# XUANTIE-RV/csi-nn2

Measured on AMD Instinct MI355X. Metric: mobilenetv1_int8_images_per_sec, higher is better.
Workload: dtype i8; 1 GPU; mobilenetv1 int8 NHWC batch 1/GPU, 28 conv layers in 15 launches, hipGraph replay via csinn_*; ops_per_image=1137480704, algorithmic_bytes_per_image=8323144, algorithmic_bytes_per_image_survey=14444616, parallelism=replicas x1

## Files before the change

csi-nn2_amd/__init__.py:

```python
import ctypes as C
import os

import numpy as np

HERE = os.path.dirname(os.path.abspath(__file__))
ROOT = os.path.dirname(HERE)
LIB_DIR = os.path.join(HERE, "lib")

DTYPE_INT8, DTYPE_INT32, DTYPE_FLOAT16, DTYPE_FLOAT32 = 3, 7, 8, 10
MEM_CPU, MEM_DMABUF, MEM_CPU_ACC = 0, 2, 5
QUANT_INT8_ASYM_W_SYM, QUANT_FLOAT16 = 11, 7
API_REF, API_GREF, API_MI355X = 0, 1, 14
RM_LAYER, RM_CPU_GRAPH = 0, 1
LAYOUT_N, LAYOUT_NC, LAYOUT_NCHW, LAYOUT_O, LAYOUT_OI, LAYOUT_OIHW, LAYOUT_O1HW = 1, 2, 4, 6, 7, 11, 13
LAYOUT_NHWC, LAYOUT_OHWI, LAYOUT_1HWO = 15, 18, 22
CSINN_TRUE = 1
OP_CONV2D, OP_CONV2D_RELU, OP_CONV2D_RELU6 = 28, 29, 30
OP_DEPTHWISE_CONV2D, OP_FULLYCONNECTED = 35, 71
OP_AVGPOOL2D, OP_MAXPOOL2D = 14, 98
OP_CONCAT = 26
OP_SPLIT, OP_SHUFFLE_CHANNEL = 166, 153
OP_SIGMOID, OP_HARD_SIGMOID, OP_SILU, OP_LEAKY_RELU, OP_MUL = 154, 78, 190, 84, 107
OP_RESIZE = 133
OP_DECONV2D, OP_DEPTHWISE_DECONV2D, OP_GROUP_DECONV2D = 54, 55, 56
# ... 158 lines not shown
                ("a_zp", C.c_int32), ("b_zp", C.c_int32), ("out_zp", C.c_int32), ("a_is_second", C.c_int32),
                ("reserved", C.c_int32 * 4)]


ABI_STRUCTS = {"csinn_quant_info": QuantInfo, "csinn_tensor": Tensor, "csinn_session": Session,
               "csinn_callback": Callback, "csinn_params_base": ParamsBase,
               "csinn_conv2d_params": Conv2dParams, "csinn_fc_params": FcParams,
               "csinn_relu_params": ReluParams, "csinn_model": Model,
               "csinn_softmax_params": SoftmaxParams, "csinn_pool_params": PoolParams,
               "csinn_diso_params": DisoParams}


def lib_path(name):
    return os.path.join(LIB_DIR, name)


_loaded = {}


def _cdll(path, mode=C.RTLD_GLOBAL):
    if path not in _loaded:
        if not os.path.exists(path):
            raise MI355XError("native library missing: %s (run python csi-nn2_amd/build.py)" % path)
        _loaded[path] = C.CDLL(path, mode=mode)
    return _loaded[path]


def load_hip():
    lib = _cdll(lib_path("libshl_mi355x.so"))
    if getattr(lib, "_typed", False):
        return lib
    vp, sz, i32, f32 = C.c_void_p, C.c_size_t, C.c_int32, C.c_float
    sigs = {
        "shl_mi355x_abi_version": (C.c_int, []),
        "shl_mi355x_last_error": (C.c_char_p, []),
        "shl_mi355x_device_count": (C.c_int, []),
        "shl_mi355x_set_device": (C.c_int, [C.c_int]),
        "shl_mi355x_device_info": (C.c_int, [C.c_char_p, sz, C.POINTER(i32), C.POINTER(C.c_int64)]),
        "shl_mi355x_malloc": (vp, [sz]),
        "shl_mi355x_free": (C.c_int, [vp]),
        "shl_mi355x_is_device_ptr": (C.c_int, [vp]),
        "shl_mi355x_upload": (C.c_int, [vp, vp, sz, vp]),
        "shl_mi355x_download": (C.c_int, [vp, vp, sz, vp]),
        "shl_mi355x_copy": (C.c_int, [vp, vp, sz, vp]),
        "shl_mi355x_memset": (C.c_int, [vp, C.c_int, sz, vp]),
        "shl_mi355x_stream_create": (vp, []),
        "shl_mi355x_stream_destroy": (C.c_int, [vp]),
        "shl_mi355x_stream_sync": (C.c_int, [vp]),
        "shl_mi355x_event_create": (vp, []),
        "shl_mi355x_event_destroy": (C.c_int, [vp]),
        "shl_mi355x_event_record": (C.c_int, [vp, vp]),
        "shl_mi355x_event_elapsed_ms": (C.c_int, [vp, vp, C.POINTER(f32)]),
        "shl_mi355x_graph_begin": (C.c_int, [vp]),
        "shl_mi355x_graph_end": (vp, [vp]),
        "shl_mi355x_graph_launch": (C.c_int, [vp, vp]),
        "shl_mi355x_graph_destroy": (C.c_int, [vp]),
        "shl_mi355x_conv_plan_create": (C.c_int, [C.POINTER(ConvDesc), vp, vp, vp, vp, C.POINTER(vp)]),
        "shl_mi355x_conv_plan_create_wzp": (C.c_int, [C.POINTER(ConvDesc), vp, vp, vp, vp, vp, C.POINTER(vp)]),
        "shl_mi355x_conv_plan_create_dw_channel": (C.c_int, [C.POINTER(ConvDesc), vp, vp, vp, vp, f32, f32, vp, C.POINTER(vp)]),
        "shl_mi355x_deconv_plan_create": (C.c_int, [C.POINTER(ConvDesc), vp, vp, vp, vp, C.POINTER(vp)]),
        "shl_mi355x_deconv_kernel_name": (C.c_char_p, [C.POINTER(ConvDesc)]),
        "shl_mi355x_deconv_geometry": (C.c_int, [C.POINTER(ConvDesc), C.POINTER(i32), i32]),
        "shl_mi355x_debug_trace": (C.c_int, [vp, i32]),
        "shl_mi355x_debug_div_check": (C.c_int, [vp, i32, vp, vp]),
        "shl_mi355x_debug_f16_round_check": (C.c_int, [vp]),
        "shl_mi355x_debug_mfma_rate": (C.c_int, [i32, i32, C.POINTER(C.c_double), C.POINTER(C.c_double)]),
        "shl_mi355x_comm_available": (C.c_int, []),
        "shl_mi355x_comm_unique_id": (C.c_int, [vp]),
        "shl_mi355x_comm_create": (C.c_int, [vp, i32, i32, C.POINTER(vp)]),
        "shl_mi355x_comm_destroy": (C.c_int, [vp]),
        "shl_mi355x_comm_info": (C.c_int, [vp, C.POINTER(i32), C.POINTER(i32), C.POINTER(i32)]),
        "shl_mi355x_device_bus_id": (C.c_int, [C.c_char_p, sz]),
        "shl_mi355x_comm_bcast": (C.c_int, [vp, C.POINTER(vp), C.POINTER(sz), i32, i32, vp]),
        "shl_mi355x_conv_plan_destroy": (C.c_int, [vp]),
        "shl_mi355x_conv_plan_algo": (C.c_int, [vp]),
        "shl_mi355x_conv_plan_kernel_name": (C.c_char_p, [vp]),
        "shl_mi355x_conv_plan_bytes": (sz, [vp]),
        "shl_mi355x_conv_plan_const_block": (vp, [vp, C.POINTER(sz)]),
        "shl_mi355x_conv_plan_adopt_block": (C.c_int, [vp, vp]),
        "shl_mi355x_conv_forward": (C.c_int, [vp, vp, vp, i32, vp]),
        "shl_mi355x_pwdw_fusable": (C.c_int, [vp, vp, i32]),
        "shl_mi355x_pwdw_form": (C.c_int, [vp, vp, i32]),
        "shl_mi355x_pwdw_geometry": (C.c_int, [vp, vp, i32, C.POINTER(i32), i32]),
        "shl_mi355x_pool_conv_fusable": (C.c_int, [vp, i32, i32]),
        "shl_mi355x_pool_conv_forward": (C.c_int, [vp, vp, vp, i32, i32, f32, i32, f32, i32, vp]),
        "shl_mi355x_conv_pool_fusable": (C.c_int, [vp, i32]),
        "shl_mi355x_conv_pool_forward": (C.c_int, [vp, vp, vp, vp, i32, f32, i32, f32, i32, vp]),
        "shl_mi355x_conv_plan_set_no_stream_consumer": (C.c_int, [vp, i32]),
        "shl_mi355x_pwdw_forward": (C.c_int, [vp, vp, vp, vp, i32, vp]),
        "shl_mi355x_relu_i8": (C.c_int, [vp, vp, sz, f32, i32, f32, i32, i32, vp]),
        "shl_mi355x_relu_f16": (C.c_int, [vp, vp, sz, i32, vp]),
        "shl_mi355x_add": (C.c_int, [vp, vp, vp, sz, i32, f32, i32, f32, i32, f32, i32, vp]),
        "shl_mi355x_layout_convert": (C.c_int, [vp, vp, C.c_int64, i32, i32, i32, i32, vp]),
        "shl_mi355x_global_avgpool2d": (C.c_int, [vp, vp, i32, i32, i32, i32, i32, f32, i32, f32, i32, vp]),
        "shl_mi355x_softmax": (C.c_int, [vp, vp, i32, C.c_int64, i32, C.c_int64, f32, i32, f32, i32, vp]),
        "shl_mi355x_pool2d": (C.c_int, [vp, vp, C.POINTER(PoolDesc), vp]),
        "shl_mi355x_pool2d_kernel_name": (C.c_char_p, [C.POINTER(PoolDesc)]),
        "shl_mi355x_concat": (C.c_int, [C.POINTER(vp), C.POINTER(C.c_int64), C.POINTER(f32), C.POINTER(i32), vp,
                                        C.POINTER(ConcatDesc), vp]),
        "shl_mi355x_concat_kernel_name": (C.c_char_p, [C.POINTER(vp), C.POINTER(C.c_int64), C.POINTER(f32), C.POINTER(i32),
                                                       vp, C.POINTER(ConcatDesc)]),
        "shl_mi355x_split": (C.c_int, [vp, C.POINTER(vp), C.POINTER(C.c_int64), C.POINTER(f32), C.POINTER(i32),
                                       C.POINTER(SplitDesc), vp]),
        "shl_mi355x_split_kernel_name": (C.c_char_p, [vp, C.POINTER(vp), C.POINTER(C.c_int64), C.POINTER(f32), C.POINTER(i32),
                                                      C.POINTER(SplitDesc)]),
        "shl_mi355x_shuffle_channel": (C.c_int, [vp, vp, C.POINTER(ShuffleDesc), vp]),
        "shl_mi355x_shuffle_channel_kernel_name": (C.c_char_p, [vp, vp, C.POINTER(ShuffleDesc)]),
        "shl_mi355x_unary_lut_i8": (C.c_int, [vp, vp, sz, vp, vp]),
        "shl_mi355x_unary_lut_i8_kernel_name": (C.c_char_p, [vp, vp]),
        "shl_mi355x_unary_f16": (C.c_int, [vp, vp, sz, i32, f32, vp]),
        "shl_mi355x_mul": (C.c_int, [vp, vp, vp, C.POINTER(MulDesc), vp]),
        "shl_mi355x_mul_kernel_name": (C.c_char_p, [C.POINTER(MulDesc), vp, vp, vp]),
        "shl_mi355x_resize": (C.c_int, [vp, vp, C.POINTER(ResizeDesc), vp]),
        "shl_mi355x_resize_kernel_name": (C.c_char_p, [C.POINTER(ResizeDesc), vp, vp]),
    }
    for name, (res, args) in sigs.items():
        fn = getattr(lib, name)
        fn.restype, fn.argtypes = res, args
    lib._typed = True
    lib.EXPORTS = sorted(sigs)
    return lib


_FRONTEND_SIGS = {
    "csinn_alloc_session": (C.POINTER(Session), []),
    "csinn_free_session": (None, [C.POINTER(Session)]),
    "csinn_session_init": (None, [C.POINTER(Session)]),
    "csinn_session_deinit": (None, [C.POINTER(Session)]),
    "csinn_session_setup": (C.c_int, [C.POINTER(Session)]),
    "csinn_session_run": (C.c_int, [C.POINTER(Session)]),
    "csinn_set_input_number": (None, [C.c_int, C.POINTER(Session)]),
    "csinn_set_output_number": (None, [C.c_int, C.POINTER(Session)]),
    "csinn_set_input": (C.c_int, [C.c_int, C.POINTER(Tensor), C.POINTER(Session)]),
    "csinn_set_output": (C.c_int, [C.c_int, C.POINTER(Tensor), C.POINTER(Session)]),
    "csinn_get_output": (C.c_int, [C.c_int, C.POINTER(Tensor), C.POINTER(Session)]),
    "csinn_update_input": (C.c_int, [C.c_int, C.POINTER(Tensor), C.POINTER(Session)]),
    "csinn_update_output": (C.c_int, [C.c_int, C.POINTER(Tensor), C.POINTER(Session)]),
    "csinn_set_tensor_entry": (C.c_int, [C.POINTER(Tensor), C.POINTER(Session)]),
    "csinn_alloc_tensor": (C.POINTER(Tensor), [C.POINTER(Session)]),
    "csinn_free_tensor": (None, [C.POINTER(Tensor)]),
    "csinn_alloc_params": (C.c_void_p, [C.c_int, C.POINTER(Session)]),
    "csinn_free_params": (None, [C.c_void_p]),
    "csinn_tensor_size": (C.c_int, [C.POINTER(Tensor)]),
    "csinn_tensor_byte_size": (C.c_int, [C.POINTER(Tensor)]),
    "shl_register_op_callback": (None, [C.c_int, C.c_void_p]),
    "shl_register_runtime_callback": (None, [C.c_int, C.c_void_p]),
    "shl_mem_alloc": (C.c_void_p, [C.c_int64]),
    "shl_mem_free": (None, [C.c_void_p]),
    "shl_debug_set_level": (None, [C.c_int]),
}
_SISO_OPS = ("csinn_relu", "csinn_relu6", "csinn_global_avgpool2d", "csinn_softmax", "csinn_maxpool2d", "csinn_avgpool2d",
             "csinn_sigmoid", "csinn_hard_sigmoid", "csinn_silu", "csinn_leaky_relu", "csinn_resize", "csinn_shuffle_channel")
_CONV_OPS = ["csinn_conv2d", "csinn_conv2d_relu", "csinn_conv2d_relu6", "csinn_depthwise_conv2d",
             "csinn_depthwise_conv2d_relu", "csinn_fullyconnected", "csinn_deconv2d"] + list(_SISO_OPS)


def load_frontend(kind="standalone", local=False, path=None):
    mode = C.RTLD_LOCAL if local else C.RTLD_GLOBAL
    if path is not None:
        lib = _cdll(path, mode)
        kind = "external"
    elif kind == "standalone":
        lib = _cdll(lib_path("libcsinn_nn2.so"), mode)
    else:
        raise ValueError(kind)
    if getattr(lib, "_typed", False):
# ... 266 lines not shown
```

csi-nn2_amd/csrc/common.h:

```cpp
#pragma once

#include <hip/hip_runtime.h>
#include <stdint.h>

#include "shl_mi355x.h"

namespace shl {

typedef int v4i __attribute__((ext_vector_type(4)));
typedef int v16i __attribute__((ext_vector_type(16)));
typedef float v16f __attribute__((ext_vector_type(16)));
typedef _Float16 v8h __attribute__((ext_vector_type(8)));

struct ConvArgs {
    const void *in;
    const void *w;
    void *out;
    const int32_t *acc_init;
    const float *mult;
    const float *bias;
    int32_t N, H, W, C;
    int32_t Ho, Wo, Co;
    int32_t Kh, Kw;
    int32_t sh, sw, pt, pl, dh, dw;
// ... 370 lines not shown
    const float c[4] = {v0, v1, v2, v3};
    uint32_t pk[8];
    finish16_f16_unit_scale<4, 0>(c, [&](int) { return bias_f; }, act, pk);
    return make_uint2(pk[0], pk[1]);
}

void set_error(const char *fmt, ...);
int hip_fail(hipError_t e, const char *what);
#define SHL_HIP(expr)                                          \
    do {                                                       \
        hipError_t e_ = (expr);                                \
        if (e_ != hipSuccess) return shl::hip_fail(e_, #expr); \
    } while (0)

struct LdsOptIn {
    unsigned long long done = 0;
};
inline void lds_opt_in(LdsOptIn &st, const void *kernel, int bytes = 160 * 1024)
{
    int dev = 0;
    if (hipGetDevice(&dev) != hipSuccess) return;
    const unsigned long long bit = 1ull << (dev & 63);
    if (__atomic_load_n(&st.done, __ATOMIC_ACQUIRE) & bit) return;
    const hipError_t e = hipFuncSetAttribute(kernel, hipFuncAttributeMaxDynamicSharedMemorySize, bytes);
    if (e != hipSuccess) {
        hip_fail(e, "hipFuncSetAttribute(MaxDynamicSharedMemorySize)");
        return;
    }
    __atomic_fetch_or(&st.done, bit, __ATOMIC_RELEASE);
}

int launch_conv_direct(const ConvArgs &a, int dtype, int layout, int dw_nhwc_weights,
                       hipStream_t s);
int launch_conv_group_direct(const ConvArgs &a, int dtype, int layout, hipStream_t s);
int launch_conv_igemm(const ConvArgs &a, int dtype, int layout, hipStream_t s);
int launch_dwconv(const ConvArgs &a, int dtype, int layout, hipStream_t s);
bool igemm_supports(const shl_mi355x_conv_desc &d);
const char *igemm_variant(int64_t M, int64_t Co, int64_t kbytes = 0);
const char *igemm_pick_name(const ConvArgs &a, int esize);
bool igemm_fuses_nchw_out(const ConvArgs &a, int esize);
bool dwconv_supports(const shl_mi355x_conv_desc &d);
bool dwconv_dot4_supports(const shl_mi355x_conv_desc &d);
void dwconv_dot4_pack(const shl_mi355x_conv_desc &d, const int8_t *hwo, uint32_t *dst);
bool dwconv_mfma_pick(int64_t M, int C, int H, int W, int Ho, int Wo, int sh, int sw);
int launch_dwconv_mfma(const ConvArgs &a, hipStream_t s);
bool conv1x1_resident_pick(const ConvArgs &a);
int launch_conv1x1_resident(const ConvArgs &a, hipStream_t s);
bool conv1x1_latency_pick(const ConvArgs &a);
int launch_conv1x1_latency(const ConvArgs &a, hipStream_t s);
bool conv1x1_pool_fusable(const ConvArgs &a);
int launch_conv1x1_pool(const ConvArgs &a, void *pool_out, float si, float zi, float so, float zo, int store_map, hipStream_t s);
bool conv1x1_stream_pick(const ConvArgs &a);
int launch_conv1x1_stream(const ConvArgs &a, hipStream_t s);
int launch_dwconv_channel(const ConvArgs &a, hipStream_t s);
bool conv_gemv_pick(const ConvArgs &a, int esize);
int launch_conv_gemv(const ConvArgs &a, int dtype, hipStream_t s);
bool pool_gemv_pick(const ConvArgs &a, int hw);
int launch_pool_gemv(const ConvArgs &a, int hw, float in_scale, int in_zp, float mid_scale, int mid_zp, hipStream_t s);
bool stem_supports(const shl_mi355x_conv_desc &d);
void stem_pack_weights(const shl_mi355x_conv_desc &d, const int8_t *ohwi, int32_t *dst);
size_t stem_weight_bytes(const shl_mi355x_conv_desc &d);
int launch_conv_stem(const ConvArgs &a, hipStream_t s);
bool conv1x1_nchw_eligible(const ConvArgs &a);
int launch_conv1x1_nchw(const ConvArgs &a, int dtype, hipStream_t s);
bool dwconv_nchw_supports(const shl_mi355x_conv_desc &d);
int launch_dwconv_nchw(const ConvArgs &a, int dtype, hipStream_t s);
bool pwdw_fusable(const ConvArgs &pw, const ConvArgs &dw, int pw_is_igemm, int dw_dot4_packed);
int launch_pwdw_fused(const ConvArgs &pw, const ConvArgs &dw, hipStream_t s);
constexpr int SHL_PWDW_GEOMETRY_FIELDS = 12;
bool pwdw_fused_geometry(const ConvArgs &pw, const ConvArgs &dw, int32_t out[SHL_PWDW_GEOMETRY_FIELDS]);
bool stemdw_f16_nchw_fusable(const ConvArgs &stem, const ConvArgs &dw);
int launch_stemdw_f16_nchw(const ConvArgs &stem, const ConvArgs &dw, hipStream_t s);
bool stem_mfma_pick(const ConvArgs &a);
bool dwpw_stream_fusable(const ConvArgs &dw, const ConvArgs &pw, int dw_dot4_packed, int pw_is_igemm);
bool dwpw_stream_takes(const ConvArgs &dw);
int launch_dwpw_stream(const ConvArgs &dw, const ConvArgs &pw, hipStream_t s);
bool dwpw_resident_fusable(const ConvArgs &dw, const ConvArgs &pw, int dw_dot4_packed, int pw_is_igemm);
bool dwpw_resident_takes(const ConvArgs &dw);
int launch_dwpw_resident(const ConvArgs &dw, const ConvArgs &pw, hipStream_t s);
bool pwdw_f16_nchw_fusable(const ConvArgs &pw, const ConvArgs &dw);
int launch_pwdw_f16_nchw(const ConvArgs &pw, const ConvArgs &dw, hipStream_t s);
bool stemdw_fusable(const ConvArgs &stem, const ConvArgs &dw);
int launch_stemdw_fused(const ConvArgs &stem, const ConvArgs &dw, hipStream_t s);
bool patch_supports(const shl_mi355x_conv_desc &d);
int patch_choose_geom(const shl_mi355x_conv_desc &d, int32_t batch);
size_t patch_weight_bytes(const shl_mi355x_conv_desc &d, int geom);
void patch_pack_weights(const shl_mi355x_conv_desc &d, int geom, const int8_t *src, int8_t *dst);
bool patch_setup(ConvArgs &a);
bool patch_auto(const ConvArgs &a, bool vs_wave = false);
int launch_conv_igemm_patch(const ConvArgs &a, hipStream_t s);
enum { DECONV_GATHER = 0, DECONV_PHASE = 1 };
const char *deconv_invalid(const shl_mi355x_conv_desc *d, int *status);
int deconv_form(const shl_mi355x_conv_desc &d, bool epilogue_ok, const char **why);
const char *deconv_form_name(int form, int dtype);
int deconv_phases(const shl_mi355x_conv_desc &d);
size_t deconv_phase_weight_bytes(const shl_mi355x_conv_desc &d);
size_t deconv_phase_acc_bytes(const shl_mi355x_conv_desc &d);
void deconv_pack_phase(const shl_mi355x_conv_desc &d, const char *ohwi, char *dst, int32_t *acc);
int launch_deconv_gather(const ConvArgs &a, int dtype, int layout, hipStream_t s);
int launch_deconv_phase(const ConvArgs &a, const shl_mi355x_conv_desc &d, hipStream_t s);
int launch_transpose(const void *src, void *dst, int64_t n, int R, int S, int esize, hipStream_t s, int to_nhwc);

}
```

csi-nn2_amd/csrc/conv_plan.hip:

```cpp
#include <stdlib.h>
#include <string.h>

#include <map>
#include <mutex>
#include <vector>

#include "igemm_common.h"

struct shl_mi355x_conv_plan {
    shl_mi355x_conv_desc desc;
    int algo;
    char *block;
    size_t block_bytes;
    size_t off_w, off_acc, off_mult, off_bias, off_pad;
    size_t off_wfrag;
    size_t off_wpatch;
    size_t off_flags;
    int32_t pt_geom;
    int32_t div_exact, div_fma, act_clamp;
    float clamp_lo, clamp_hi, inv_out_scale;
    char *scratch_in, *scratch_out;
    int2 *pix_tab;
    float ch_in_scale, ch_out_scale;
    int32_t ch_has_bias;
// ... 1044 lines not shown
    if (a.M == 0) return SHL_MI355X_OK;
    return launch_pool_gemv(a, pixels, in_scale, in_zp, mid_scale, mid_zp, (hipStream_t)stream);
}

int shl_mi355x_conv_pool_fusable(const shl_mi355x_conv_plan *plan, int32_t batch)
{
    using namespace shl;
    if (!plan || batch <= 0) return 0;
    const char *sel = getenv("SHL_MI355X_CONVPOOL");
    if (sel && sel[0] == '0') return 0;
    if (plan->desc.dtype != SHL_MI355X_I8 || plan->desc.layout != SHL_MI355X_NHWC || plan->algo != SHL_MI355X_ALGO_IGEMM) return 0;
    if (igemm_env_override()) return 0;
    ConvArgs a;
    static char dummy[16];
    if (fill_args(plan, dummy, dummy, batch, a) != SHL_MI355X_OK) return 0;
    return conv1x1_pool_fusable(a) ? 1 : 0;
}

int shl_mi355x_conv_pool_forward(const shl_mi355x_conv_plan *plan, const void *input_dev, void *map_dev, void *pool_dev, int32_t batch,
                                 float mid_scale, int32_t mid_zp, float out_scale, int32_t out_zp, void *stream)
{
    using namespace shl;
    if (!plan || !input_dev || !pool_dev) {
        set_error("conv_pool_forward: NULL argument");
        return SHL_MI355X_EINVAL;
    }
    if (!shl_mi355x_conv_pool_fusable(plan, batch)) {
        set_error("conv_pool_forward: the pair does not qualify for the fused kernel");
        return SHL_MI355X_ENOTSUP;
    }
    ConvArgs a;
    static char dummy[16];
    int rc = fill_args(plan, input_dev, map_dev ? map_dev : dummy, batch, a);
    if (rc != SHL_MI355X_OK) return rc;
    if (a.M == 0) return SHL_MI355X_OK;
    return launch_conv1x1_pool(a, pool_dev, mid_scale, (float)mid_zp, out_scale, (float)out_zp, map_dev ? 1 : 0, (hipStream_t)stream);
}

int shl_mi355x_pwdw_form(const shl_mi355x_conv_plan *pw, const shl_mi355x_conv_plan *dw, int32_t batch)
{
    if (!dw || !pw || is_deconv(pw) || is_deconv(dw)) return 0;
    static const char *off = getenv("SHL_MI355X_NO_FUSION");
    static const char *sel = getenv("SHL_MI355X_PWDW");
    if ((off && off[0] == '1') || (sel && sel[0] == '0')) return 0;
    if (dw->desc.dtype != pw->desc.dtype || dw->desc.layout != pw->desc.layout) return 0;
    const bool i8_nhwc = pw->desc.dtype == SHL_MI355X_I8 && pw->desc.layout == SHL_MI355X_NHWC;
    const bool f16_nchw = pw->desc.dtype == SHL_MI355X_F16 && pw->desc.layout == SHL_MI355X_NCHW;
    if (!i8_nhwc && !f16_nchw) return 0;
    ConvArgs a, b;
    static char dummy[16];
    if (fill_args(pw, dummy, dummy, batch, a) != SHL_MI355X_OK || fill_args(dw, dummy, dummy, batch, b) != SHL_MI355X_OK)
        return 0;
    return pwdw_kernel_for(pw, dw, a, b);
}

int shl_mi355x_pwdw_fusable(const shl_mi355x_conv_plan *pw, const shl_mi355x_conv_plan *dw, int32_t batch)
{
    return shl_mi355x_pwdw_form(pw, dw, batch) ? 1 : 0;
}

int shl_mi355x_pwdw_geometry(const shl_mi355x_conv_plan *pw, const shl_mi355x_conv_plan *dw, int32_t batch, int32_t *out, int32_t count)
{
    using namespace shl;
    if (!out || count < SHL_PWDW_GEOMETRY_FIELDS) {
        set_error("pwdw_geometry: room for 12 values is needed");
        return SHL_MI355X_EINVAL;
    }
    if (shl_mi355x_pwdw_form(pw, dw, batch) != 1) {
        set_error("pwdw_geometry: the pair does not run the latency form");
        return SHL_MI355X_ENOTSUP;
    }
    ConvArgs a, b;
    static char dummy[16];
    int rc = fill_args(pw, dummy, dummy, batch, a);
    if (rc == SHL_MI355X_OK) rc = fill_args(dw, dummy, dummy, batch, b);
    if (rc != SHL_MI355X_OK) return rc;
    if (!pwdw_fused_geometry(a, b, out)) {
        set_error("pwdw_geometry: the pair does not qualify");
        return SHL_MI355X_ENOTSUP;
    }
    return SHL_MI355X_OK;
}

int shl_mi355x_pwdw_forward(const shl_mi355x_conv_plan *pw, const shl_mi355x_conv_plan *dw, const void *input_dev,
                            void *output_dev, int32_t batch, void *stream)
{
    if (!dw || !pw || !input_dev || !output_dev) {
        set_error("pwdw_forward: NULL argument");
        return SHL_MI355X_EINVAL;
    }
    if (!shl_mi355x_pwdw_fusable(pw, dw, batch)) {
        set_error("pwdw_forward: the pair does not qualify for the fused kernel");
        return SHL_MI355X_ENOTSUP;
    }
    ConvArgs a, b;
    int rc = fill_args(pw, input_dev, output_dev, batch, a);
    if (rc == SHL_MI355X_OK) rc = fill_args(dw, input_dev, output_dev, batch, b);
    if (rc != SHL_MI355X_OK) return rc;
    if (b.M == 0) return SHL_MI355X_OK;
    switch (pwdw_kernel_for(pw, dw, a, b)) {
        case 7: return launch_dwpw_resident(a, b, (hipStream_t)stream);
        case 6: return launch_dwpw_stream(a, b, (hipStream_t)stream);
        case 5: return launch_stemdw_f16_nchw(a, b, (hipStream_t)stream);
        case 4: return launch_pwdw_f16_nchw(a, b, (hipStream_t)stream);
        case 3: return launch_stemdw_fused(a, b, (hipStream_t)stream);
        default: return launch_pwdw_fused(a, b, (hipStream_t)stream);
    }
}

}
```

csi-nn2_amd/csrc/stemdw_fused.hip:

```cpp
#include <stdio.h>
#include <stdlib.h>

#include "dw_patch.h"

namespace shl {

struct StemDwArgs {
    ConvArgs st;
    ConvArgs dw;
    int32_t bh, bw;
    int32_t tiles_x, tiles_y;
    int32_t rw, npx;
    uint32_t rw_magic, bw_magic;
};

template <int EPQ, int EPD>
__global__ __launch_bounds__(256) void stemdw_fused_kernel(StemDwArgs f)
{
    extern __shared__ __attribute__((aligned(16))) char smem[];
    const ConvArgs &q = f.st;
    const ConvArgs &d = f.dw;
    asm volatile("" ::"s"(q.in), "s"(q.w), "s"(q.acc_init), "s"(q.mult), "s"(q.bias), "s"(q.H), "s"(q.W), "s"(q.Ho), "s"(q.Wo), "s"(q.sh),
                 "s"(q.sw), "s"(q.pt), "s"(q.pl), "s"(q.dh), "s"(q.dw), "s"(q.in_zp));
    asm volatile("" ::"s"(f.bh), "s"(f.bw), "s"(f.tiles_y), "s"(f.rw), "s"(f.npx), "s"(f.rw_magic), "s"(f.bw_magic), "s"(d.N), "s"(d.sh),
                 "s"(d.sw), "s"(d.pt), "s"(d.pl), "s"(d.w), "s"(d.acc_init), "s"(d.mult), "s"(d.bias), "s"(d.out));
    asm volatile("" ::"s"(q.out_zp), "s"(q.out_zp_f), "s"(q.clamp_lo), "s"(q.clamp_hi), "s"(d.out_zp), "s"(d.out_zp_f), "s"(d.clamp_lo),
                 "s"(d.clamp_hi), "s"(d.in_zp), "s"(d.Ho), "s"(d.Wo), "s"(d.H), "s"(d.W), "s"(d.C));
    const int tid = threadIdx.x;
    int32_t *w_lds = reinterpret_cast<int32_t *>(smem);
    int32_t *t_tab = w_lds + 7 * 32;
    uint32_t *patch = reinterpret_cast<uint32_t *>(t_tab + 96);
    if (tid < 224) w_lds[tid] = static_cast<const int32_t *>(q.w)[tid];
    if (tid < 96) {
        const int which = tid >> 5, i = tid & 31;
        t_tab[tid] = which == 0 ? q.acc_init[i] : which == 1 ? __float_as_int(q.mult[i]) : __float_as_int(q.bias[i]);
    }
    const int tx = blockIdx.x;
    int ty = blockIdx.y, n = 0;
    if (d.N > 1) {
        n = ty / f.tiles_y;
        ty -= n * f.tiles_y;
    }
    const int oy0 = ty * f.bh, ox0 = tx * f.bw;
    const int ry0 = oy0 * d.sh - d.pt, rx0 = ox0 * d.sw - d.pl;
    const DwThreadConsts dwk = dw_load_consts(d, 0, tid);

    const int8_t *img = static_cast<const int8_t *>(q.in) + (int64_t)n * q.H * q.W * 3;
    const int ntasks = 2 * f.npx;
    const int ppitch = dw_patch_pitch(f.npx);
    const uint32_t zpad = dw_patch_pad(d);
    DwPatchGeom g;
    g.bh = f.bh, g.bw = f.bw, g.rw = f.rw, g.bw_magic = f.bw_magic, g.pitch = ppitch;
    g.lbh = min(f.bh, d.Ho - oy0), g.lbw = min(f.bw, d.Wo - ox0);
    g.oy0 = oy0, g.ox0 = ox0, g.ry0 = ry0, g.rx0 = rx0, g.n = n, g.ch0 = 0;
    const DwPrep dwp = dw_patch_prepare(d, g, tid);
    for (int base = 0; base < ntasks; base += 256) {
        const bool valid = base + tid < ntasks;
        const int task = valid ? base + tid : ntasks - 1;
        const int j = task >> 1, cb = (task & 1) * 16;
        const int pr = (int)(((uint32_t)j * f.rw_magic) >> 20);
        const int pc = j - pr * f.rw;
        const int sy = ry0 + pr, sx = rx0 + pc;
        const bool inside = (unsigned)sy < (unsigned)q.Ho && (unsigned)sx < (unsigned)q.Wo;
        const int y0 = sy * q.sh - q.pt, x0 = sx * q.sw - q.pl;
        int qv[28];
#pragma unroll
        for (int ky = 0; ky < 3; ++ky)
#pragma unroll
            for (int kx = 0; kx < 3; ++kx) {
                const int y = y0 + ky * q.dh, x = x0 + kx * q.dw;
                const bool ok = inside && (unsigned)y < (unsigned)q.H && (unsigned)x < (unsigned)q.W;
                const int8_t *px = img + ((int64_t)y * q.W + x) * 3;
#pragma unroll
                for (int c = 0; c < 3; ++c) qv[(ky * 3 + kx) * 3 + c] = ok ? (int)px[c] : q.in_zp;
            }
        qv[27] = 0;
        uint32_t q4[7];
#pragma unroll
        for (int g = 0; g < 7; ++g)
            q4[g] = (uint32_t)(qv[4 * g] & 0xFF) | ((uint32_t)(qv[4 * g + 1] & 0xFF) << 8) |
                    ((uint32_t)(qv[4 * g + 2] & 0xFF) << 16) | ((uint32_t)(qv[4 * g + 3] & 0xFF) << 24);
        if (base == 0) __syncthreads();
        int acc[16];
#pragma unroll
        for (int e = 0; e < 16; ++e) acc[e] = 0;
#pragma unroll
        for (int g = 0; g < 7; ++g)
#pragma unroll
            for (int v = 0; v < 4; ++v) {
                const int4 w = *reinterpret_cast<const int4 *>(&w_lds[g * 32 + cb + 4 * v]);
                acc[4 * v + 0] = __builtin_amdgcn_sdot4((int)q4[g], w.x, acc[4 * v + 0], false);
                acc[4 * v + 1] = __builtin_amdgcn_sdot4((int)q4[g], w.y, acc[4 * v + 1], false);
                acc[4 * v + 2] = __builtin_amdgcn_sdot4((int)q4[g], w.z, acc[4 * v + 2], false);
                acc[4 * v + 3] = __builtin_amdgcn_sdot4((int)q4[g], w.w, acc[4 * v + 3], false);
            }
#pragma unroll
        for (int v = 0; v < 4; ++v) {
            const int c = cb + 4 * v;
            const int4 ai = *reinterpret_cast<const int4 *>(t_tab + c);
            const float4 mu = *reinterpret_cast<const float4 *>(t_tab + 32 + c);
            const float4 bi = *reinterpret_cast<const float4 *>(t_tab + 64 + c);
            const uint32_t pk = requant4_i8_sel<EPQ>(acc[4 * v] + ai.x, acc[4 * v + 1] + ai.y, acc[4 * v + 2] + ai.z,
                                               acc[4 * v + 3] + ai.w, mu, bi, q);
            if (valid) patch[dw_patch_slot(j, c >> 2, ppitch)] = inside ? pk : zpad;
        }
    }
    __syncthreads();

    depthwise_from_patch<EPD>(d, patch, g, dwk, dwp, tid, 256);
}

static bool stemdw_geometry(const ConvArgs &q, const ConvArgs &d, StemDwArgs &f)
{
    if (q.Kh != 3 || q.Kw != 3 || q.C != 3 || q.Co != 32) return false;
    if (d.Kh != 3 || d.Kw != 3 || d.dh != 1 || d.dw != 1 || d.C != 32 || d.Co != 32) return false;
    if (d.H != q.Ho || d.W != q.Wo || d.N != q.N || d.sh < 1 || d.sh > 2 || d.sw < 1 || d.sw > 2) return false;
    if (d.pt < 0 || d.pl < 0 || d.pt > 2 || d.pl > 2) return false;
    if ((int64_t)d.Ho * d.Wo * d.C >= ((int64_t)1 << 31)) return false;
    f.bh = d.Ho < 2 ? d.Ho : 2;
    f.bw = d.Wo < 28 ? d.Wo : 28;
    if (const char *e = getenv("SHL_MI355X_STEMDW_TILE")) {
        int h = 0, w = 0;
        if (sscanf(e, "%dx%d", &h, &w) == 2 && h > 0 && w > 0) f.bh = h < d.Ho ? h : d.Ho, f.bw = w < d.Wo ? w : d.Wo;
    }
    f.tiles_y = (d.Ho + f.bh - 1) / f.bh;
    f.tiles_x = (d.Wo + f.bw - 1) / f.bw;
    f.rw = (f.bw - 1) * d.sw + 3;
    f.npx = ((f.bh - 1) * d.sh + 3) * f.rw;
    f.rw_magic = ((1u << 20) + f.rw - 1) / f.rw;
    f.bw_magic = ((1u << 20) + f.bw - 1) / f.bw;
    if (f.npx >= 2048 || f.tiles_x > 65535 || (int64_t)f.tiles_y * d.N > 65535) return false;
    return (int64_t)f.tiles_x * f.tiles_y * d.N <= 2048;
}

bool stemdw_fusable(const ConvArgs &q, const ConvArgs &d)
{
    StemDwArgs f;
    return stemdw_geometry(q, d, f);
}

int launch_stemdw_fused(const ConvArgs &q, const ConvArgs &d, hipStream_t s)
{
    StemDwArgs f;
    f.st = q;
    f.dw = d;
    if (!stemdw_geometry(q, d, f)) {
        set_error("stemdw_fused: the pair does not qualify");
        return SHL_MI355X_ENOTSUP;
    }
    const dim3 grid((unsigned)f.tiles_x, (unsigned)(f.tiles_y * d.N));
    const size_t lds = (size_t)(7 * 32 + 96) * 4 + dw_patch_bytes(f.npx);
    const int epq = (q.act != SHL_MI355X_ACT_NONE && !q.act_clamp) ? -1 : (q.div_exact ? 3 : 0);
    const int epd = (d.act != SHL_MI355X_ACT_NONE && !d.act_clamp) ? -1 : (d.div_exact ? 3 : 0);
    if (epq == 3 && epd == 3) hipLaunchKernelGGL((stemdw_fused_kernel<3, 3>), grid, dim3(256), lds, s, f);
    else if (epq == 0 && epd == 0) hipLaunchKernelGGL((stemdw_fused_kernel<0, 0>), grid, dim3(256), lds, s, f);
    else hipLaunchKernelGGL((stemdw_fused_kernel<-1, -1>), grid, dim3(256), lds, s, f);
    SHL_HIP(hipGetLastError());
    return SHL_MI355X_OK;
}

}
```

include/shl_mi355x.h:

```cpp
#ifndef SHL_MI355X_H_
#define SHL_MI355X_H_

#include <stddef.h>
#include <stdint.h>

#ifdef __cplusplus
extern "C" {
#endif

#define SHL_MI355X_ABI_VERSION 1

enum shl_mi355x_status {
    SHL_MI355X_OK = 0,
    SHL_MI355X_ENODEV = -1,
    SHL_MI355X_EINVAL = -2,
    SHL_MI355X_ENOTSUP = -3,
    SHL_MI355X_EHIP = -4,
    SHL_MI355X_ENOMEM = -5
};

enum shl_mi355x_layout {
    SHL_MI355X_NHWC = 0,
    SHL_MI355X_NCHW = 1
};
// ... 42 lines not shown

typedef struct shl_mi355x_conv_plan shl_mi355x_conv_plan;

int shl_mi355x_abi_version(void);
const char *shl_mi355x_last_error(void);
int shl_mi355x_device_count(void);
int shl_mi355x_set_device(int ordinal);
int shl_mi355x_device_info(char *arch, size_t arch_len, int32_t *cu_count, int64_t *hbm_bytes);
int shl_mi355x_device_bus_id(char *buf, size_t len);

void *shl_mi355x_malloc(size_t bytes);
int shl_mi355x_free(void *ptr_dev);
int shl_mi355x_is_device_ptr(const void *ptr);
int shl_mi355x_upload(void *dst_dev, const void *src_host, size_t bytes, void *stream);
int shl_mi355x_download(void *dst_host, const void *src_dev, size_t bytes, void *stream);
int shl_mi355x_copy(void *dst_dev, const void *src_dev, size_t bytes, void *stream);
int shl_mi355x_memset(void *dst_dev, int byte_value, size_t bytes, void *stream);
void *shl_mi355x_stream_create(void);
int shl_mi355x_stream_destroy(void *stream);
int shl_mi355x_stream_sync(void *stream);

void *shl_mi355x_event_create(void);
int shl_mi355x_event_destroy(void *event);
int shl_mi355x_event_record(void *event, void *stream);
int shl_mi355x_event_elapsed_ms(void *start, void *stop, float *ms);

int shl_mi355x_graph_begin(void *stream);
void *shl_mi355x_graph_end(void *stream);
int shl_mi355x_graph_launch(void *graph_exec, void *stream);
int shl_mi355x_graph_destroy(void *graph_exec);


int shl_mi355x_conv_plan_create(const struct shl_mi355x_conv_desc *desc,
                                const void *kernel_host, const float *mult_host,
                                const float *bias_host, void *stream,
                                shl_mi355x_conv_plan **plan_out);
int shl_mi355x_conv_plan_create_wzp(const struct shl_mi355x_conv_desc *desc, const void *kernel_host,
                                    const float *mult_host, const float *bias_host, const int32_t *kernel_zp,
                                    void *stream, shl_mi355x_conv_plan **plan_out);
int shl_mi355x_comm_available(void);
int shl_mi355x_comm_unique_id(void *id128);
int shl_mi355x_comm_create(const void *id128, int32_t rank, int32_t world, void **comm_out);
int shl_mi355x_comm_destroy(void *comm);
int shl_mi355x_comm_info(void *comm, int32_t *nranks, int32_t *rank, int32_t *device);
int shl_mi355x_comm_bcast(void *comm, void *const *blocks_dev, const size_t *bytes, int32_t count, int32_t root,
                          void *stream);

int shl_mi355x_debug_trace(uint64_t *host, int32_t count);

int shl_mi355x_debug_div_check(const float *divisors_host, int32_t n, uint64_t *mismatches, float *first_pair);
int shl_mi355x_debug_f16_round_check(uint64_t *out3);
int shl_mi355x_debug_mfma_rate(int32_t form, int32_t waves_per_simd, double *tops, double *ns_per_mfma);

int shl_mi355x_conv_plan_create_dw_channel(const struct shl_mi355x_conv_desc *desc, const void *kernel_host,
                                           const float *kernel_scale, const int32_t *kernel_zp,
                                           const int32_t *bias_i32, float in_scale, float out_scale_ms,
                                           void *stream, shl_mi355x_conv_plan **plan_out);

int shl_mi355x_deconv_plan_create(const struct shl_mi355x_conv_desc *desc, const void *kernel_host, const float *mult_host,
                                  const float *bias_host, void *stream, shl_mi355x_conv_plan **plan_out);
const char *shl_mi355x_deconv_kernel_name(const struct shl_mi355x_conv_desc *desc);
int shl_mi355x_deconv_geometry(const struct shl_mi355x_conv_desc *desc, int32_t *out, int32_t count);

int shl_mi355x_conv_plan_destroy(shl_mi355x_conv_plan *plan);
int shl_mi355x_conv_plan_algo(const shl_mi355x_conv_plan *plan);
const char *shl_mi355x_conv_plan_kernel_name(const shl_mi355x_conv_plan *plan);
size_t shl_mi355x_conv_plan_bytes(const shl_mi355x_conv_plan *plan);
void *shl_mi355x_conv_plan_const_block(shl_mi355x_conv_plan *plan, size_t *bytes);
int shl_mi355x_conv_plan_adopt_block(shl_mi355x_conv_plan *plan, void *stream);

int shl_mi355x_conv_forward(const shl_mi355x_conv_plan *plan, const void *input_dev,
                            void *output_dev, int32_t batch, void *stream);

int shl_mi355x_pool_conv_fusable(const shl_mi355x_conv_plan *plan, int32_t batch, int32_t pixels);
int shl_mi355x_pool_conv_forward(const shl_mi355x_conv_plan *plan, const void *input_dev, void *output_dev, int32_t batch,
                                 int32_t pixels, float in_scale, int32_t in_zp, float mid_scale, int32_t mid_zp, void *stream);
int shl_mi355x_conv_pool_fusable(const shl_mi355x_conv_plan *plan, int32_t batch);
int shl_mi355x_conv_pool_forward(const shl_mi355x_conv_plan *plan, const void *input_dev, void *map_dev, void *pool_dev, int32_t batch,
                                 float mid_scale, int32_t mid_zp, float out_scale, int32_t out_zp, void *stream);
int shl_mi355x_conv_plan_set_no_stream_consumer(shl_mi355x_conv_plan *plan, int32_t on);
int shl_mi355x_pwdw_fusable(const shl_mi355x_conv_plan *pw, const shl_mi355x_conv_plan *dw, int32_t batch);
int shl_mi355x_pwdw_form(const shl_mi355x_conv_plan *pw, const shl_mi355x_conv_plan *dw, int32_t batch);
int shl_mi355x_pwdw_geometry(const shl_mi355x_conv_plan *pw, const shl_mi355x_conv_plan *dw, int32_t batch, int32_t *out, int32_t count);
int shl_mi355x_pwdw_forward(const shl_mi355x_conv_plan *pw, const shl_mi355x_conv_plan *dw,
                            const void *input_dev, void *output_dev, int32_t batch, void *stream);

int shl_mi355x_relu_i8(const int8_t *input_dev, int8_t *output_dev, size_t count,
                       float in_scale, int32_t in_zp, float out_scale, int32_t out_zp,
                       int32_t relu6, void *stream);

int shl_mi355x_relu_f16(const uint16_t *input_dev, uint16_t *output_dev, size_t count, int32_t relu6,
                        void *stream);

int shl_mi355x_add(const void *input0_dev, const void *input1_dev, void *output_dev, size_t count,
                   int32_t dtype, float scale0, int32_t zp0, float scale1, int32_t zp1, float out_scale,
                   int32_t out_zp, void *stream);

int shl_mi355x_global_avgpool2d(const void *input_dev, void *output_dev, int32_t dtype, int32_t layout,
                                int32_t batch, int32_t channels, int32_t pixels, float in_scale,
                                int32_t in_zp, float out_scale, int32_t out_zp, void *stream);

enum shl_mi355x_pool_kind {
    SHL_MI355X_POOL_MAX = 0,
    SHL_MI355X_POOL_AVG = 1
};

struct shl_mi355x_pool_desc {
    int32_t kind;
    int32_t dtype;
    int32_t layout;
    int32_t batch, c, in_h, in_w, out_h, out_w;
    int32_t kernel_h, kernel_w, stride_h, stride_w, pad_top, pad_left;
    int32_t count_include_pad;
    int32_t in_zp, out_zp;
    float in_scale, out_scale;
    int32_t reserved[4];
};

int shl_mi355x_pool2d(const void *in_dev, void *out_dev, const struct shl_mi355x_pool_desc *d, void *stream);
const char *shl_mi355x_pool2d_kernel_name(const struct shl_mi355x_pool_desc *d);

struct shl_mi355x_concat_desc {
    int32_t dtype;
    int32_t n_inputs;
    int64_t outer;
    float out_scale;
    int32_t out_zp;
    int32_t reserved[4];
};

int shl_mi355x_concat(const void *const *in_dev, const int64_t *len, const float *in_scale, const int32_t *in_zp,
                      void *out_dev, const struct shl_mi355x_concat_desc *d, void *stream);
const char *shl_mi355x_concat_kernel_name(const void *const *in_dev, const int64_t *len, const float *in_scale,
                                          const int32_t *in_zp, const void *out_dev,
                                          const struct shl_mi355x_concat_desc *d);

struct shl_mi355x_split_desc {
    int32_t dtype;
    int32_t n_outputs;
    int64_t outer;
    float in_scale;
    int32_t in_zp;
    int32_t reserved[4];
};

int shl_mi355x_split(const void *in_dev, void *const *out_dev, const int64_t *len, const float *out_scale,
                     const int32_t *out_zp, const struct shl_mi355x_split_desc *d, void *stream);
const char *shl_mi355x_split_kernel_name(const void *in_dev, void *const *out_dev, const int64_t *len, const float *out_scale,
                                         const int32_t *out_zp, const struct shl_mi355x_split_desc *d);

struct shl_mi355x_shuffle_desc {
    int32_t dtype;
    int32_t group;
    int64_t outer, c, inner;
    float in_scale;
    int32_t in_zp;
    float out_scale;
    int32_t out_zp;
    int32_t reserved[4];
};

int shl_mi355x_shuffle_channel(const void *in_dev, void *out_dev, const struct shl_mi355x_shuffle_desc *d, void *stream);
const char *shl_mi355x_shuffle_channel_kernel_name(const void *in_dev, const void *out_dev,
                                                   const struct shl_mi355x_shuffle_desc *d);

enum shl_mi355x_resize_mode {
// ... 60 lines not shown
```

Baseline: 19480 img/s.

## Stage raw stem input rows in LDS for fused stem+depthwise kernel

```diff
diff --git a/csi-nn2_amd/__init__.py b/csi-nn2_amd/__init__.py
--- a/csi-nn2_amd/__init__.py
+++ b/csi-nn2_amd/__init__.py
@@ -264,6 +264,7 @@
         "shl_mi355x_pwdw_fusable": (C.c_int, [vp, vp, i32]),
         "shl_mi355x_pwdw_form": (C.c_int, [vp, vp, i32]),
         "shl_mi355x_pwdw_geometry": (C.c_int, [vp, vp, i32, C.POINTER(i32), i32]),
+        "shl_mi355x_stemdw_geometry": (C.c_int, [vp, vp, i32, vp, C.POINTER(i32), i32]),
         "shl_mi355x_pool_conv_fusable": (C.c_int, [vp, i32, i32]),
         "shl_mi355x_pool_conv_forward": (C.c_int, [vp, vp, vp, i32, i32, f32, i32, f32, i32, vp]),
         "shl_mi355x_conv_pool_fusable": (C.c_int, [vp, i32]),
diff --git a/csi-nn2_amd/csrc/common.h b/csi-nn2_amd/csrc/common.h
--- a/csi-nn2_amd/csrc/common.h
+++ b/csi-nn2_amd/csrc/common.h
@@ -476,6 +476,8 @@
 int launch_pwdw_f16_nchw(const ConvArgs &pw, const ConvArgs &dw, hipStream_t s);
 bool stemdw_fusable(const ConvArgs &stem, const ConvArgs &dw);
 int launch_stemdw_fused(const ConvArgs &stem, const ConvArgs &dw, hipStream_t s);
+constexpr int SHL_STEMDW_GEOMETRY_FIELDS = 12;
+bool stemdw_fused_geometry(const ConvArgs &stem, const ConvArgs &dw, int32_t out[SHL_STEMDW_GEOMETRY_FIELDS]);
 bool patch_supports(const shl_mi355x_conv_desc &d);
 int patch_choose_geom(const shl_mi355x_conv_desc &d, int32_t batch);
 size_t patch_weight_bytes(const shl_mi355x_conv_desc &d, int geom);
diff --git a/csi-nn2_amd/csrc/conv_plan.hip b/csi-nn2_amd/csrc/conv_plan.hip
--- a/csi-nn2_amd/csrc/conv_plan.hip
+++ b/csi-nn2_amd/csrc/conv_plan.hip
@@ -1150,6 +1150,30 @@
     return SHL_MI355X_OK;
 }
 
+int shl_mi355x_stemdw_geometry(const shl_mi355x_conv_plan *stem, const shl_mi355x_conv_plan *dw, int32_t batch, const void *input_dev,
+                               int32_t *out, int32_t count)
+{
+    using namespace shl;
+    if (!out || count < SHL_STEMDW_GEOMETRY_FIELDS) {
+        set_error("stemdw_geometry: room for 12 values is needed");
+        return SHL_MI355X_EINVAL;
+    }
+    if (shl_mi355x_pwdw_form(stem, dw, batch) != 3) {
+        set_error("stemdw_geometry: the pair does not run the stem + depthwise form");
+        return SHL_MI355X_ENOTSUP;
+    }
+    ConvArgs a, b;
+    alignas(16) static char dummy[16];
+    int rc = fill_args(stem, input_dev ? input_dev : dummy, dummy, batch, a);
+    if (rc == SHL_MI355X_OK) rc = fill_args(dw, dummy, dummy, batch, b);
+    if (rc != SHL_MI355X_OK) return rc;
+    if (!stemdw_fused_geometry(a, b, out)) {
+        set_error("stemdw_geometry: the pair does not qualify");
+        return SHL_MI355X_ENOTSUP;
+    }
+    return SHL_MI355X_OK;
+}
+
 int shl_mi355x_pwdw_forward(const shl_mi355x_conv_plan *pw, const shl_mi355x_conv_plan *dw, const void *input_dev,
                             void *output_dev, int32_t batch, void *stream)
 {
diff --git a/csi-nn2_amd/csrc/stemdw_fused.hip b/csi-nn2_amd/csrc/stemdw_fused.hip
--- a/csi-nn2_amd/csrc/stemdw_fused.hip
+++ b/csi-nn2_amd/csrc/stemdw_fused.hip
@@ -1,3 +1,4 @@
+#include <stdint.h>
 #include <stdio.h>
 #include <stdlib.h>
 
@@ -110,6 +111,211 @@
     depthwise_from_patch<EPD>(d, patch, g, dwk, dwp, tid, 256);
 }
 
+
+struct alignas(64) StemStageEarly {
+    const void *in;
+    int32_t H;
+    int32_t w3;
+    int32_t img;
+    int32_t N, tiles_y;
+    int32_t ystep, yoff;
+    int32_t xstep, xoff;
+    int32_t ndw;
+    uint32_t ndw_magic;
+    int32_t nstage;
+    int32_t reserved[2];
+};
+
+struct StemDwStageArgs {
+    StemStageEarly e;
+    StemDwArgs f;
+    int32_t qsw3;
+    int32_t ih, iw;
+};
+
+template <int THREADS, int CPT, bool ONEPASS, int EPQ, int EPD>
+__global__ __launch_bounds__(THREADS) void stemdw_staged_kernel(StemDwStageArgs a)
+{
+    constexpr int NLD = 512 / THREADS;
+    constexpr int TSH = CPT == 16 ? 1 : 2;
+    constexpr int NV = CPT / 4;
+    static_assert((CPT == 16 || CPT == 8) && (THREADS == 256 || THREADS == 512), "stemdw_staged: 256 x 16 or 512 x 8");
+    extern __shared__ __attribute__((aligned(16))) char smem[];
+    const StemStageEarly &e = a.e;
+    asm volatile("" ::"s"(e.in), "s"(e.H), "s"(e.w3), "s"(e.img), "s"(e.N), "s"(e.tiles_y), "s"(e.ystep), "s"(e.yoff), "s"(e.xstep),
+                 "s"(e.xoff), "s"(e.ndw), "s"(e.ndw_magic), "s"(e.nstage));
+    const int tid = threadIdx.x;
+    const int tx = blockIdx.x;
+    int ty = blockIdx.y, n = 0;
+    if (e.N > 1) {
+        n = ty / e.tiles_y;
+        ty -= n * e.tiles_y;
+    }
+    const int iy0 = ty * e.ystep - e.yoff;
+    const int bx0 = tx * e.xstep - e.xoff;
+    const int rlo0 = n * e.img + iy0 * e.w3;
+    const int t0 = rlo0 + bx0;
+    auto stage_request = [&](int i, uint32_t &v, int &lo, bool &need) {
+        const int r = (int)(((uint32_t)i * e.ndw_magic) >> 20);
+        const int k = i - r * e.ndw;
+        const int rlo = rlo0 + r * e.w3;
+        const int o0 = ((rlo + bx0) & ~3) + 4 * k;
+        lo = rlo - o0;
+        need = i < e.nstage && (unsigned)(iy0 + r) < (unsigned)e.H && lo < 4 && lo + e.w3 > 0;
+        v = 0;
+        if (need) v = *reinterpret_cast<const uint32_t *>(static_cast<const char *>(e.in) + o0);
+    };
+    auto stage_blend = [&](uint32_t v, int lo, bool need, uint32_t zp4) {
+        const int b0 = max(lo, 0), b1 = min(lo + e.w3, 4);
+        const uint32_t m = need ? (0xffffffffu << (8 * b0)) & (0xffffffffu >> (8 * (4 - b1))) : 0u;
+        return (v & m) | (zp4 & ~m);
+    };
+    uint32_t sv[NLD];
+    int slo[NLD];
+    bool sneed[NLD];
+#pragma unroll
+    for (int l = 0; l < NLD; ++l) stage_request(tid + l * THREADS, sv[l], slo[l], sneed[l]);
+
+    __builtin_amdgcn_sched_barrier(0);
+    const StemDwArgs f = kernarg_here<StemDwArgs>(offsetof(StemDwStageArgs, f));
+    const int qsw3 = kernarg_here<int32_t>(offsetof(StemDwStageArgs, qsw3));
+    const ConvArgs &q = f.st;
+    const ConvArgs &d = f.dw;
+    asm volatile("" ::"s"(q.w), "s"(q.acc_init), "s"(q.mult), "s"(q.bias), "s"(q.Ho), "s"(q.Wo), "s"(q.sh), "s"(q.in_zp), "s"(qsw3),
+                 "s"(q.out_zp), "s"(q.out_zp_f), "s"(q.clamp_lo), "s"(q.clamp_hi), "s"(q.out_scale), "s"(q.inv_out_scale));
+    asm volatile("" ::"s"(f.bh), "s"(f.bw), "s"(f.rw), "s"(f.npx), "s"(f.rw_magic), "s"(f.bw_magic), "s"(d.sh), "s"(d.sw), "s"(d.pt),
+                 "s"(d.pl), "s"(d.w), "s"(d.acc_init), "s"(d.mult), "s"(d.bias), "s"(d.out));
+    asm volatile("" ::"s"(d.out_zp), "s"(d.out_zp_f), "s"(d.clamp_lo), "s"(d.clamp_hi), "s"(d.out_scale), "s"(d.inv_out_scale),
+                 "s"(d.in_zp), "s"(d.Ho), "s"(d.Wo), "s"(d.C));
+    int32_t *w_lds = reinterpret_cast<int32_t *>(smem);
+    int32_t *t_tab = w_lds + 7 * 32;
+    uint32_t *patch = reinterpret_cast<uint32_t *>(t_tab + 96);
+    const int wi = min(tid, 223), ti = min(tid, 95);
+    const int32_t wv = static_cast<const int32_t *>(q.w)[wi];
+    const int32_t *tsrc = ti < 32 ? q.acc_init : ti < 64 ? reinterpret_cast<const int32_t *>(q.mult) - 32 : reinterpret_cast<const int32_t *>(q.bias) - 64;
+    const int32_t tv = tsrc[ti];
+    const DwThreadConsts dwk = dw_load_consts(d, 0, tid);
+    const int oy0 = ty * f.bh, ox0 = tx * f.bw;
+    const int ry0 = oy0 * d.sh - d.pt, rx0 = ox0 * d.sw - d.pl;
+    const int ntasks = f.npx << TSH;
+    const int ppitch = dw_patch_pitch(f.npx);
+    const uint32_t zpad = dw_patch_pad(d);
+    const uint32_t zp4 = (uint32_t)(q.in_zp & 0xff) * 0x01010101u;
+    uint32_t *stage = patch + 8 * ppitch;
+    DwPatchGeom g;
+    g.bh = f.bh, g.bw = f.bw, g.rw = f.rw, g.bw_magic = f.bw_magic, g.pitch = ppitch;
+    g.lbh = min(f.bh, d.Ho - oy0), g.lbw = min(f.bw, d.Wo - ox0);
+    g.oy0 = oy0, g.ox0 = ox0, g.ry0 = ry0, g.rx0 = rx0, g.n = n, g.ch0 = 0;
+    const DwPrep dwp = dw_patch_prepare(d, g, tid);
+    {
+        const float qcl = q.clamp_lo - q.out_zp_f, qch = q.clamp_hi - q.out_zp_f, dcl = d.clamp_lo - d.out_zp_f, dch = d.clamp_hi - d.out_zp_f;
+        const uint32_t qzp2 = (uint32_t)(q.out_zp & 0xffff) * 0x00010001u, dzp2 = (uint32_t)(d.out_zp & 0xffff) * 0x00010001u;
+        asm volatile("" ::"s"(ppitch), "s"(zpad), "s"(zp4), "v"(qcl), "v"(qch), "v"(dcl), "v"(dch), "s"(qzp2), "s"(dzp2));
+    }
+    struct Task {
+        uint32_t at[3], ph[3];
+        uint32_t slot;
+        uint32_t inside;
+        int cb;
+    };
+    auto locate = [&](int task) {
+        Task t;
+        const int j = task >> TSH;
+        t.cb = (task & ((1 << TSH) - 1)) * CPT;
+        const int pr = (int)(((uint32_t)j * f.rw_magic) >> 20);
+        const int pc = j - pr * f.rw;
+        const int sy = ry0 + pr, sx = rx0 + pc;
+        t.inside = ((unsigned)sy < (unsigned)q.Ho && (unsigned)sx < (unsigned)q.Wo) ? 1u : 0u;
+        const int r0 = pr * q.sh, b0 = pc * qsw3;
+#pragma unroll
+        for (int ky = 0; ky < 3; ++ky) {
+            const int r = r0 + ky;
+            const int b = ((t0 + r * e.w3) & 3) + b0;
+            t.at[ky] = (uint32_t)(r * e.ndw + (b >> 2));
+            t.ph[ky] = (uint32_t)(b & 3);
+        }
+        t.slot = (uint32_t)dw_patch_slot(j, t.cb >> 2, ppitch);
+        return t;
+    };
+    Task t1;
+    if constexpr (ONEPASS) {
+        const bool valid = tid < ntasks;
+        t1 = locate(valid ? tid : ntasks - 1);
+        t1.slot = valid ? t1.slot : (uint32_t)((t1.cb >> 2) * ppitch + ppitch - 1);
+        asm volatile("" ::"v"(t1.at[0]), "v"(t1.at[1]), "v"(t1.at[2]), "v"(t1.ph[0]), "v"(t1.ph[1]), "v"(t1.ph[2]), "v"(t1.slot), "v"(t1.inside));
+    }
+    __builtin_amdgcn_sched_barrier(0);
+
+#pragma unroll
+    for (int l = 0; l < NLD; ++l) stage[tid + l * THREADS] = stage_blend(sv[l], slo[l], sneed[l], zp4);
+    w_lds[wi] = wv;
+    t_tab[ti] = tv;
+    if constexpr (!ONEPASS) {
+        for (int i = tid + NLD * THREADS; i < e.nstage; i += THREADS) {
+            uint32_t v;
+            int lo;
+            bool need;
+            stage_request(i, v, lo, need);
+            stage[i] = stage_blend(v, lo, need, zp4);
+        }
+    }
+    __syncthreads();
+
+    auto run = [&](const Task &t, bool valid) {
+        uint32_t e0[3], e1[3], e2[3];
+#pragma unroll
+        for (int ky = 0; ky < 3; ++ky) {
+            const uint32_t *p = stage + t.at[ky];
+            const uint32_t a0 = p[0], a1 = p[1], a2 = p[2];
+            e0[ky] = __builtin_amdgcn_alignbyte(a1, a0, t.ph[ky]);
+            e1[ky] = __builtin_amdgcn_alignbyte(a2, a1, t.ph[ky]);
+            e2[ky] = __builtin_amdgcn_alignbyte(a2, a2, t.ph[ky]);
+        }
+        uint32_t q4[7];
+        q4[0] = e0[0];
+        q4[1] = e1[0];
+        q4[2] = __builtin_amdgcn_perm(e0[1], e2[0], 0x06050400u);
+        q4[3] = __builtin_amdgcn_alignbyte(e1[1], e0[1], 3);
+        q4[4] = __builtin_amdgcn_perm(e0[2], __builtin_amdgcn_perm(e2[1], e1[1], 0x0c0c0403u), 0x05040100u);
+        q4[5] = __builtin_amdgcn_alignbyte(e1[2], e0[2], 2);
+        q4[6] = __builtin_amdgcn_perm(e2[2], e1[2], 0x0c040302u);
+        int acc[CPT];
+#pragma unroll
+        for (int c = 0; c < CPT; ++c) acc[c] = 0;
+#pragma unroll
+        for (int k4 = 0; k4 < 7; ++k4)
+#pragma unroll
+            for (int v = 0; v < NV; ++v) {
+                const int4 w = *reinterpret_cast<const int4 *>(&w_lds[k4 * 32 + t.cb + 4 * v]);
+                acc[4 * v + 0] = __builtin_amdgcn_sdot4((int)q4[k4], w.x, acc[4 * v + 0], false);
+                acc[4 * v + 1] = __builtin_amdgcn_sdot4((int)q4[k4], w.y, acc[4 * v + 1], false);
+                acc[4 * v + 2] = __builtin_amdgcn_sdot4((int)q4[k4], w.z, acc[4 * v + 2], false);
+                acc[4 * v + 3] = __builtin_amdgcn_sdot4((int)q4[k4], w.w, acc[4 * v + 3], false);
+            }
+#pragma unroll
+        for (int v = 0; v < NV; ++v) {
+            const int c = t.cb + 4 * v;
+            const int4 ai = *reinterpret_cast<const int4 *>(t_tab + c);
+            const float4 mu = *reinterpret_cast<const float4 *>(t_tab + 32 + c);
+            const float4 bi = *reinterpret_cast<const float4 *>(t_tab + 64 + c);
+            const uint32_t pk = requant4_i8_sel<EPQ>(acc[4 * v] + ai.x, acc[4 * v + 1] + ai.y, acc[4 * v + 2] + ai.z,
+                                               acc[4 * v + 3] + ai.w, mu, bi, q);
+            if (ONEPASS || valid) patch[t.slot + v * ppitch] = t.inside ? pk : zpad;
+        }
+    };
+    if constexpr (ONEPASS) {
+        run(t1, true);
+    } else {
+        for (int base = 0; base < ntasks; base += THREADS) {
+            const bool valid = base + tid < ntasks;
+            run(locate(valid ? base + tid : ntasks - 1), valid);
+        }
+    }
+    __syncthreads();
+
+    depthwise_from_patch<EPD>(d, patch, g, dwk, dwp, tid, THREADS);
+}
+
 static bool stemdw_geometry(const ConvArgs &q, const ConvArgs &d, StemDwArgs &f)
 {
     if (q.Kh != 3 || q.Kw != 3 || q.C != 3 || q.Co != 32) return false;
@@ -139,6 +345,65 @@
     return stemdw_geometry(q, d, f);
 }
 
+static bool stemdw_stage_geometry(const ConvArgs &q, const ConvArgs &d, const StemDwArgs &f, StemDwStageArgs &a, int &threads, bool &onepass,
+                                  size_t &lds)
+{
+    const char *sw = getenv("SHL_MI355X_STEMDW_STAGE");
+    if (sw && sw[0] == '0') return false;
+    const int64_t total = (int64_t)q.N * q.H * q.W * 3;
+    if ((reinterpret_cast<uintptr_t>(q.in) & 3) != 0 || (total & 3) != 0) return false;
+    if (q.dh != 1 || q.dw != 1 || q.sh < 1 || q.sh > 2 || q.sw < 1 || q.sw > 2 || q.pt < 0 || q.pl < 0) return false;
+    const int rh = (f.bh - 1) * d.sh + 3;
+    const int ih = (rh - 1) * q.sh + 3, iw = (f.rw - 1) * q.sw + 3;
+    const int ndw = (3 * iw + 6) / 4;
+    const int nstage = ih * ndw;
+    if (ndw >= 256 || nstage > 4096) return false;
+    const int64_t ymax = (int64_t)(f.tiles_y - 1) * f.bh * d.sh * q.sh + ih, xmax = (int64_t)(f.tiles_x - 1) * f.bw * d.sw * q.sw + iw;
+    if (total + (ymax + 8) * q.W * 3 + (xmax + 8) * 3 >= ((int64_t)1 << 31)) return false;
+    threads = 512;
+    if (const char *t = getenv("SHL_MI355X_STEMDW_THREADS")) {
+        if (atoi(t) == 256) threads = 256;
+        if (atoi(t) == 512) threads = 512;
+    }
+    const int ntasks = f.npx * (threads == 256 ? 2 : 4);
+    onepass = ntasks <= threads && nstage <= 512;
+    lds = (size_t)(7 * 32 + 96) * 4 + dw_patch_bytes(f.npx) + (size_t)(nstage > 512 ? nstage : 512) * 4;
+    if (lds > 64 * 1024) return false;
+    a.f = f;
+    a.e.in = q.in;
+    a.e.H = q.H, a.e.w3 = q.W * 3, a.e.img = q.H * q.W * 3;
+    a.e.N = q.N, a.e.tiles_y = f.tiles_y;
+    a.e.ystep = f.bh * d.sh * q.sh, a.e.yoff = d.pt * q.sh + q.pt;
+    a.e.xstep = f.bw * d.sw * q.sw * 3, a.e.xoff = (d.pl * q.sw + q.pl) * 3;
+    a.e.ndw = ndw, a.e.ndw_magic = ((1u << 20) + ndw - 1) / ndw, a.e.nstage = nstage;
+    a.e.reserved[0] = a.e.reserved[1] = 0;
+    a.qsw3 = 3 * q.sw;
+    a.ih = ih, a.iw = iw;
+    return true;
+}
+
+bool stemdw_fused_geometry(const ConvArgs &q, const ConvArgs &d, int32_t out[SHL_STEMDW_GEOMETRY_FIELDS])
+{
+    StemDwArgs f;
+    f.st = q;
+    f.dw = d;
+    if (!stemdw_geometry(q, d, f)) return false;
+    StemDwStageArgs a;
+    int threads = 256;
+    bool onepass = false;
+    size_t lds = 0;
+    const bool staged = stemdw_stage_geometry(q, d, f, a, threads, onepass, lds);
+    if (!staged) threads = 256;
+    const int cpt = threads == 256 ? 16 : 8;
+    const int ntasks = f.npx * (32 / cpt);
+    const int rh = (f.bh - 1) * d.sh + 3;
+    const int32_t v[SHL_STEMDW_GEOMETRY_FIELDS] = {staged ? 1 : 0, threads, cpt, (ntasks + threads - 1) / threads, staged ? a.e.nstage * 4 : 0,
+                                                   f.tiles_y, f.tiles_x, f.bh, f.bw,
+                                                   (rh - 1) * q.sh + 3, (f.rw - 1) * q.sw + 3, staged ? a.e.ndw : 0};
+    for (int i = 0; i < SHL_STEMDW_GEOMETRY_FIELDS; ++i) out[i] = v[i];
+    return true;
+}
+
 int launch_stemdw_fused(const ConvArgs &q, const ConvArgs &d, hipStream_t s)
 {
     StemDwArgs f;
@@ -149,9 +414,31 @@
         return SHL_MI355X_ENOTSUP;
     }
     const dim3 grid((unsigned)f.tiles_x, (unsigned)(f.tiles_y * d.N));
-    const size_t lds = (size_t)(7 * 32 + 96) * 4 + dw_patch_bytes(f.npx);
     const int epq = (q.act != SHL_MI355X_ACT_NONE && !q.act_clamp) ? -1 : (q.div_exact ? 3 : 0);
     const int epd = (d.act != SHL_MI355X_ACT_NONE && !d.act_clamp) ? -1 : (d.div_exact ? 3 : 0);
+    StemDwStageArgs a;
+    int threads = 256;
+    bool onepass = false;
+    size_t slds = 0;
+    if (stemdw_stage_geometry(q, d, f, a, threads, onepass, slds)) {
+#define SHL_STEMDW_EPI(THREADS, CPT, ONE)                                                                               \
+    do {                                                                                                                \
+        if (epq == 3 && epd == 3) hipLaunchKernelGGL((stemdw_staged_kernel<THREADS, CPT, ONE, 3, 3>), grid, dim3(THREADS), slds, s, a);      \
+        else if (epq == 0 && epd == 0) hipLaunchKernelGGL((stemdw_staged_kernel<THREADS, CPT, ONE, 0, 0>), grid, dim3(THREADS), slds, s, a); \
+        else hipLaunchKernelGGL((stemdw_staged_kernel<THREADS, CPT, ONE, -1, -1>), grid, dim3(THREADS), slds, s, a);    \
+    } while (0)
+        if (threads == 512) {
+            if (onepass) SHL_STEMDW_EPI(512, 8, true);
+            else SHL_STEMDW_EPI(512, 8, false);
+        } else {
+            if (onepass) SHL_STEMDW_EPI(256, 16, true);
+            else SHL_STEMDW_EPI(256, 16, false);
+        }
+#undef SHL_STEMDW_EPI
+        SHL_HIP(hipGetLastError());
+        return SHL_MI355X_OK;
+    }
+    const size_t lds = (size_t)(7 * 32 + 96) * 4 + dw_patch_bytes(f.npx);
     if (epq == 3 && epd == 3) hipLaunchKernelGGL((stemdw_fused_kernel<3, 3>), grid, dim3(256), lds, s, f);
     else if (epq == 0 && epd == 0) hipLaunchKernelGGL((stemdw_fused_kernel<0, 0>), grid, dim3(256), lds, s, f);
     else hipLaunchKernelGGL((stemdw_fused_kernel<-1, -1>), grid, dim3(256), lds, s, f);
diff --git a/include/shl_mi355x.h b/include/shl_mi355x.h
--- a/include/shl_mi355x.h
+++ b/include/shl_mi355x.h
@@ -148,6 +148,8 @@
 int shl_mi355x_pwdw_fusable(const shl_mi355x_conv_plan *pw, const shl_mi355x_conv_plan *dw, int32_t batch);
 int shl_mi355x_pwdw_form(const shl_mi355x_conv_plan *pw, const shl_mi355x_conv_plan *dw, int32_t batch);
 int shl_mi355x_pwdw_geometry(const shl_mi355x_conv_plan *pw, const shl_mi355x_conv_plan *dw, int32_t batch, int32_t *out, int32_t count);
+int shl_mi355x_stemdw_geometry(const shl_mi355x_conv_plan *stem, const shl_mi355x_conv_plan *dw, int32_t batch, const void *input_dev,
+                               int32_t *out, int32_t count);
 int shl_mi355x_pwdw_forward(const shl_mi355x_conv_plan *pw, const shl_mi355x_conv_plan *dw,
                             const void *input_dev, void *output_dev, int32_t batch, void *stream);
 
```

Result: no change. 19390 img/s (-0.5%).
